# NoahVl/Explaining-In-Style-Reproducibility-Study

Hardware: AMD Instinct MI355X
Metric: StylEx G+D+enc train-step images/sec @256px (higher is better)
Workload: dtype bf16; 1 GPU; FFHQ-shaped 256x256 StylEx, batch 32/GPU, GAE=2 (noise+encoder micro-steps), GP every 4th step, ResNet-18 classifier; image_size=256, batch_per_gpu=32, start_step=0, gradient_accumulate_every=2, global_batch=32, parallelism=dp1

## Files before the change

### explaining-in-style-reproducibility-study_amd/csrc/conv_pipe.hip

```cpp
#include <hip/hip_runtime.h>
#include <stdint.h>
#include <stdlib.h>

#include "conv_prims.h"
#include "stylex_internal.h"

#ifndef PIPE_STORE_AUX
#define PIPE_STORE_AUX 0
#endif

struct StylexPipeArgs {
    int total_tiles;
    unsigned m_ntiles, m_tpi, m_tx;
    int dbg;
};

#ifdef STYLEX_PIPE_ABLATION
#define PIPE_DBG (pa.dbg)
#else
#define PIPE_DBG 0
#endif


namespace {

typedef StylexPipeArgs PipeArgs;

template <int NT>
struct PipeCfg {
    static constexpr int TH = NT == 128 ? 16 : 32;
    static constexpr int TW = 32, HWD = TW + 2, NP = (TH + 2) * HWD;
    static constexpr int H_PIECES = (NP + 31) / 32;
    static constexpr int H_STRIDE = H_PIECES * 1024;
    static constexpr int W_PIECES = 9 * NT / 32;
    static constexpr int W_STRIDE = W_PIECES * 1024;
    static constexpr int HS = 3, WS = 2;
    static constexpr int W_BASE = HS * H_STRIDE;
    static constexpr int BIAS_BASE = W_BASE + WS * W_STRIDE;
    static constexpr int DUMP_BASE = BIAS_BASE + 2048;
    static constexpr int SMEM = DUMP_BASE + 1024;
    static constexpr int HP_MAX = (H_PIECES + 7) / 8;
    static constexpr int WP_MAX = (W_PIECES + 7) / 8;
    static constexpr int RG = TH / 4;
};

__device__ __forceinline__ void lds_wait(bf16x8 (&av)[4], bf16x8 (&bv)[2]) {
    asm volatile("s_waitcnt lgkmcnt(0)" : "+v"(av[0]), "+v"(av[1]), "+v"(av[2]), "+v"(av[3]), "+v"(bv[0]), "+v"(bv[1]));
}
template <int HWD, int TAP>
__device__ __forceinline__ void tap_addr(int (&addr)[4], int a_base, unsigned& swz) {
    constexpr int kh = TAP / 3, kw = TAP % 3;
    asm volatile("" : "+v"(swz));
#pragma unroll
    for (int i = 0; i < 4; ++i) addr[i] = a_base + ((i + kh) * HWD + kw) * 32 + (int)(((swz >> ((i + kh) * 3 + kw)) & 1u) << 4);
}
template <int NT, int TAP>
__device__ __forceinline__ void load_tap(bf16x8 (&av)[4], bf16x8 (&bv)[2], const int (&addr)[4], int b_addr) {
    lds_read16<(TAP * NT) * 32>(bv[0], b_addr);
    lds_read16<(TAP * NT + 32) * 32>(bv[1], b_addr);
#pragma unroll
    for (int i = 0; i < 4; ++i) lds_read16<0>(av[i], addr[i]);
}

__device__ __forceinline__ void mfma8(f32x16 (&acc)[4][2], const bf16x8 (&av)[4], const bf16x8 (&bv)[2]) {
#pragma unroll
    for (int i = 0; i < 4; ++i)
#pragma unroll
        for (int j = 0; j < 2; ++j) mfma1(acc[i][j], bv[j], av[i]);
}

template <int NT, int EPI>
__global__ __launch_bounds__(512, 2) void conv3x3_pipe_kernel(ConvKParams p, PipeArgs pa) {
    using Cfg = PipeCfg<NT>;
    constexpr int TH = Cfg::TH, HWD = Cfg::HWD, NP = Cfg::NP, H_PIECES = Cfg::H_PIECES, H_STRIDE = Cfg::H_STRIDE;
    constexpr int W_PIECES = Cfg::W_PIECES, W_STRIDE = Cfg::W_STRIDE, W_BASE = Cfg::W_BASE;
    constexpr int HP_MAX = Cfg::HP_MAX, WP_MAX = Cfg::WP_MAX, RG = Cfg::RG;
    static_assert(WP_MAX + HP_MAX <= 9, "one DMA piece per tap");
    extern __shared__ __attribute__((aligned(16))) char smem[];
    const int tid = threadIdx.x, lane = tid & 63;
    const int wave = __builtin_amdgcn_readfirstlane(tid >> 6);
    const int H = p.Ho, W = p.Wo, C = p.Ck, N = p.N;
    const int n_tiles = N / NT;
    const int tiles_x = (W + 31) >> 5, tiles_y = (H + TH - 1) / TH;
    const int tpi = tiles_x * tiles_y;

    int xs, xn, bslot, nslots;
    xcd_tile_span(pa.total_tiles, xs, xn, bslot, nslots);
    if (bslot >= xn) return;
    for (int i = (bslot & 3) * (PIPE_DBG >> 8); i > 0; --i) __builtin_amdgcn_s_sleep(16);
    const int my_tiles = xcd_my_tiles(xn, bslot, nslots);
    const int nchunks = C >> 4;
    const int total = my_tiles * nchunks;

    auto decode = [&](int k, int& b, int& y0, int& x0, int& n0) {
        const int t = xs + bslot + k * nslots;
        int pt = fastdiv(t, pa.m_ntiles);
        n0 = (t - pt * n_tiles) * NT;
        b = fastdiv(pt, pa.m_tpi);
        pt -= b * tpi;
        const int ty = fastdiv(pt, pa.m_tx);
        y0 = ty * TH;
        x0 = (pt - ty * tiles_x) * 32;
    };

    const unsigned bytes_x = (unsigned)((long)p.B * H * W * C * 2);
    const unsigned bytes_w = (unsigned)((long)N * 9 * C * 2);
    const __amdgpu_buffer_rsrc_t rx = __builtin_amdgcn_make_buffer_rsrc(const_cast<float*>(p.a), 0, (int)bytes_x, 0x00020000);
    const __amdgpu_buffer_rsrc_t rw = __builtin_amdgcn_make_buffer_rsrc(const_cast<void*>(p.w), 0, (int)bytes_w, 0x00020000);
    constexpr unsigned OOB = 0x80000000u;

    const int lr = lane >> 1, pslot = lane & 1;
    const int half = pslot ^ ((lr >> 3) & 1);
    int h_dst[HP_MAX], w_dst[WP_MAX];
#pragma unroll
    for (int it = 0; it < HP_MAX; ++it) h_dst[it] = wave + 8 * it < H_PIECES ? (wave + 8 * it) * 1024 : -1;
    unsigned voff_h[HP_MAX];
    auto halo_voff = [&](int b, int y0, int x0) {
#pragma unroll
        for (int it = 0; it < HP_MAX; ++it) {
            const int piece = wave + 8 * it;
            const int hp = piece * 32 + lr;
            const int hh = hp / HWD, ww = hp - hh * HWD;
            const int y = y0 - 1 + hh, x = x0 - 1 + ww;
            const bool ok = piece < H_PIECES && hp < NP && y >= 0 && y < H && x >= 0 && x < W;
            voff_h[it] = ok ? ((unsigned)((b * H + y) * W + x) * (unsigned)C + (unsigned)half * 8u) * 2u : OOB;
        }
    };
    unsigned voff_w[WP_MAX];
#pragma unroll
    for (int it = 0; it < WP_MAX; ++it) {
        const int piece = wave + 8 * it;
        const int r = piece * 32 + lr;
        const int tap = r / NT, n = r - tap * NT;
        const int gt = p.flip_taps ? 8 - tap : tap;
        voff_w[it] = piece < W_PIECES ? ((unsigned)(n * 9 + gt) * (unsigned)C + (unsigned)half * 8u) * 2u : OOB;
        w_dst[it] = piece < W_PIECES ? piece * 1024 : -1;
    }
#define issue_h1(IT, STAGE, SOFF, MORE)                                                                              \
    dma16(rx, smem, h_dst[IT] >= 0 ? (STAGE) * H_STRIDE + h_dst[IT] : Cfg::DUMP_BASE, (MORE) ? voff_h[IT] : OOB, SOFF)
#define issue_w1(IT, WBUF, SOFF, MORE)                                                                               \
    dma16(rw, smem, w_dst[IT] >= 0 ? W_BASE + (WBUF) * W_STRIDE + w_dst[IT] : Cfg::DUMP_BASE, (MORE) ? voff_w[IT] : OOB, SOFF)

    const int rg = wave % RG, nh = wave / RG;
    const int li = lane & 31, lk = lane >> 5;
    const int a_row = (4 * rg) * HWD + li;
    int a_base = a_row * 32;
    unsigned swz = 0;
#pragma unroll
    for (int r = 0; r < 6; ++r)
#pragma unroll
        for (int kw = 0; kw < 3; ++kw) {
            const int t = a_row + r * HWD + kw;
            swz |= (unsigned)(((t >> 3) ^ lk) & 1) << (r * 3 + kw);
        }
    const int b_cur0 = W_BASE + (nh * 64 + li) * 32 + ((((li >> 3) ^ lk) & 1) << 4), b_cur1 = b_cur0 + W_STRIDE;

    if (EPI == 0 && (p.flags & STYLEX_EPI_BIAS) && tid < N) reinterpret_cast<float*>(smem + Cfg::BIAS_BASE)[tid] = p.bias[tid];

    f32x16 acc[4][2];
    auto zero_acc = [&]() {
#pragma unroll
        for (int i = 0; i < 4; ++i)
#pragma unroll
            for (int j = 0; j < 2; ++j)
#pragma unroll
                for (int e = 0; e < 16; ++e) acc[i][j][e] = 0.f;
    };
    zero_acc();

    const bool act = EPI == 0 && (p.flags & (STYLEX_EPI_LRELU | STYLEX_EPI_RELU)) != 0;
    const float slope = (p.flags & STYLEX_EPI_RELU) ? 0.f : 0.2f;
    const float gslope = p.res_scale;
    const bool mask_out = EPI == 0 && p.mask != nullptr;
    auto gatem = [&](unsigned u, unsigned bits) -> unsigned {
        const float a0 = __uint_as_float(u << 16), c0 = __uint_as_float(u & 0xffff0000u);
        f32x2_t t = {(bits & 1u) ? a0 : gslope * a0, (bits & 2u) ? c0 : gslope * c0};
        bf16x2_t r = __builtin_convertvector(t, bf16x2_t);
        return *reinterpret_cast<unsigned*>(&r);
    };
    auto gate2 = [&](unsigned u, unsigned g) -> unsigned {
        const float a0 = __uint_as_float(u << 16), c0 = __uint_as_float(u & 0xffff0000u);
        const float ga = __uint_as_float(g << 16), gc = __uint_as_float(g & 0xffff0000u);
        f32x2_t t = {ga > 0.f ? a0 : gslope * a0, gc > 0.f ? c0 : gslope * c0};
        bf16x2_t r = __builtin_convertvector(t, bf16x2_t);
        return *reinterpret_cast<unsigned*>(&r);
    };
    const unsigned bytes_y = (unsigned)((long)p.B * H * W * N * 2);
    const __amdgpu_buffer_rsrc_t ry = __builtin_amdgcn_make_buffer_rsrc(p.y, 0, (int)bytes_y, 0x00020000);
    const __amdgpu_buffer_rsrc_t rgate = __builtin_amdgcn_make_buffer_rsrc(const_cast<float*>(p.residual), 0, (int)bytes_y, 0x00020000);
    const __amdgpu_buffer_rsrc_t rmask = __builtin_amdgcn_make_buffer_rsrc(
        EPI == 2 ? const_cast<unsigned char*>(p.gate_mask) : p.mask, 0, (int)(bytes_y >> 4), 0x00020000);
    const unsigned rowb = (unsigned)(W * N) * 2u;
    auto pack2 = [](float a, float c) -> unsigned {
        f32x2_t t = {a, c};
        bf16x2_t r = __builtin_convertvector(t, bf16x2_t);
        return *reinterpret_cast<unsigned*>(&r);
    };
    const unsigned lane_off = (unsigned)(((4 * rg) * W + (lane & 7)) * N + nh * 64) * 2u +
                              (unsigned)(4 * ((lane >> 4) & 1) + 2 * ((lane >> 3) & 1) + (lane >> 5)) * 16u;
    const unsigned pixb8 = (unsigned)N * 16u;
    auto epilogue = [&](int b, int y0, int x0, int n0) {
        const int lh = lk;
        const int nb = n0 + nh * 64;
        const unsigned t_off = __builtin_amdgcn_readfirstlane((unsigned)((((long)(b * H + y0) * W + x0) * N + n0) * 2));
        const unsigned g_off = x0 + li < W ? (unsigned)(((4 * rg) * W + li) * N + nh * 64 + 8 * lh) * 2u : OOB;
#pragma unroll
        for (int i = 0; i < 4; ++i) {
            const bool row_ok = y0 + 4 * rg + i < H;
            const unsigned soff = t_off + i * rowb;
            u32x4 R[4];
#pragma unroll
            for (int j = 0; j < 2; ++j) {
                u32x4 gv[2];
                unsigned gm[2];
                if (EPI != 0) {
                    const unsigned voff = row_ok ? g_off : OOB;
#pragma unroll
                    for (int q = 0; q < 2; ++q) {
                        if (EPI == 1) gv[q] = __builtin_amdgcn_raw_buffer_load_b128(rgate, voff + (j * 64 + q * 32), soff, 0);
                        if (EPI == 2) gm[q] = __builtin_amdgcn_raw_buffer_load_b8(rmask, (voff >> 4) + (j * 4 + q * 2), soff >> 4, 0);
                    }
                }
                float4 b4[4];
#pragma unroll
                for (int g = 0; g < 4; ++g)
                    b4[g] = (EPI == 0 && (p.flags & STYLEX_EPI_BIAS))
                                ? *reinterpret_cast<const float4*>(smem + Cfg::BIAS_BASE + (nb + j * 32 + 8 * g + 4 * lh) * 4)
                                : make_float4(0.f, 0.f, 0.f, 0.f);
                unsigned P[4][2];
#pragma unroll
                for (int g = 0; g < 4; ++g) {
                    float v0 = acc[i][j][4 * g + 0] + b4[g].x, v1 = acc[i][j][4 * g + 1] + b4[g].y;
                    float v2 = acc[i][j][4 * g + 2] + b4[g].z, v3 = acc[i][j][4 * g + 3] + b4[g].w;
                    if (act) {
                        v0 = v0 > 0.f ? v0 : slope * v0;
                        v1 = v1 > 0.f ? v1 : slope * v1;
                        v2 = v2 > 0.f ? v2 : slope * v2;
                        v3 = v3 > 0.f ? v3 : slope * v3;
                    }
                    P[g][0] = pack2(v0, v1);
                    P[g][1] = pack2(v2, v3);
                }
#pragma unroll
                for (int g = 0; g < 4; g += 2)
#pragma unroll
                    for (int h = 0; h < 2; ++h) {
                        auto r = __builtin_amdgcn_permlane32_swap(P[g][h], P[g + 1][h], false, false);
                        P[g][h] = r[0];
                        P[g + 1][h] = r[1];
                    }
#pragma unroll
                for (int q = 0; q < 2; ++q) {
                    uint4 v = make_uint4(P[2 * q][0], P[2 * q][1], P[2 * q + 1][0], P[2 * q + 1][1]);
                    if (EPI == 1) {
                        v.x = gate2(v.x, gv[q].x);
                        v.y = gate2(v.y, gv[q].y);
                        v.z = gate2(v.z, gv[q].z);
                        v.w = gate2(v.w, gv[q].w);
                    } else if (EPI == 2) {
                        const unsigned m = gm[q];
                        v.x = gatem(v.x, m);
                        v.y = gatem(v.y, m >> 2);
                        v.z = gatem(v.z, m >> 4);
                        v.w = gatem(v.w, m >> 6);
                    }
                    if (mask_out && !(PIPE_DBG & 1))
                        __builtin_amdgcn_raw_buffer_store_b8((unsigned char)stylex_sign_bits8(v), rmask,
                                                             ((row_ok ? g_off : OOB) >> 4) + (j * 4 + q * 2), soff >> 4, 0);
                    R[2 * j + q] = u32x4{v.x, v.y, v.z, v.w};
                }
            }
#pragma unroll
            for (int j = 0; j < 2; ++j)
#pragma unroll
                for (int d = 0; d < 4; ++d) {
                    const unsigned a0 = R[2 * j][d], a1 = R[2 * j + 1][d];
                    R[2 * j][d] = (unsigned)__builtin_amdgcn_update_dpp((int)a0, (int)a1, 0x128, 0xF, 0xC, false);
                    R[2 * j + 1][d] = (unsigned)__builtin_amdgcn_update_dpp((int)a1, (int)a0, 0x128, 0xF, 0x3, false);
                }
#pragma unroll
            for (int q = 0; q < 2; ++q)
#pragma unroll
                for (int d = 0; d < 4; ++d) {
                    auto r = __builtin_amdgcn_permlane16_swap(R[q][d], R[2 + q][d], false, false);
                    R[q][d] = r[0];
                    R[2 + q][d] = r[1];
                }
            if (!(PIPE_DBG & 1)) {
#pragma unroll
                for (int k = 0; k < 4; ++k) {
                    const unsigned voff = (row_ok && x0 + 8 * k + (lane & 7) < W) ? lane_off : OOB;
                    __builtin_amdgcn_raw_buffer_store_b128(R[k], ry, voff, soff + k * pixb8, PIPE_STORE_AUX);
                    asm volatile("s_nop 1" : "+v"(R[k]) : : "memory");
                }
            }
        }
    };

    int hb, hy0, hx0, hn0;
    int h_k = 0, h_ch = 0, h_stage = 0;
    int w_k = 0, w_ch = 0, w_buf = 0, w_n0;
    int cb, cy0, cx0, cn0;
    decode(0, cb, cy0, cx0, cn0);
    hb = cb, hy0 = cy0, hx0 = cx0, hn0 = cn0;
    w_n0 = cn0;
    halo_voff(hb, hy0, hx0);
    auto adv_h = [&]() {
        h_stage = h_stage == 2 ? 0 : h_stage + 1;
        if (++h_ch == nchunks) {
            h_ch = 0;
            if (++h_k < my_tiles) {
                decode(h_k, hb, hy0, hx0, hn0);
                if (PIPE_DBG & 2) hb = 0, hy0 = 0, hx0 = 0;
                halo_voff(hb, hy0, hx0);
            }
        }
    };
    auto adv_w = [&]() {
        w_buf ^= 1;
        if (++w_ch == nchunks) {
            w_ch = 0;
            if (++w_k < my_tiles) {
                int b_, y_, x_;
                decode(w_k, b_, y_, x_, w_n0);
                if (PIPE_DBG & 4) w_n0 = 0;
            }
        }
    };
#pragma unroll
    for (int it = 0; it < HP_MAX; ++it) issue_h1(it, 0, 0u, true);
    adv_h();
#pragma unroll
    for (int it = 0; it < WP_MAX; ++it) issue_w1(it, 0, (unsigned)(w_n0 * 9 * C) * 2u, true);
    adv_w();
#pragma unroll
    for (int it = 0; it < HP_MAX; ++it) issue_h1(it, 1, (unsigned)h_ch * 32u, total > 1);
    if (total > 1) adv_h();

    int c_ch = 0, c_k = 0, c_stage = 0;
    bf16x8 avA[4], bvA[2], avB[4], bvB[2];
    int addr[4];
    tap_addr<HWD, 0>(addr, a_base, swz);
    wait_vmcnt<HP_MAX>();
    __builtin_amdgcn_s_barrier();
    asm volatile("" ::: "memory");
    load_tap<NT, 0>(avA, bvA, addr, b_cur0);
    tap_addr<HWD, 1>(addr, a_base, swz);
    auto next_stage = [&]() {
        a_base += c_stage == 2 ? -2 * H_STRIDE : H_STRIDE;
        c_stage = c_stage == 2 ? 0 : c_stage + 1;
    };
    constexpr int PPT = 2;
#define PIPE_DMA(TAP, MORE_W, MORE_H)                                                              \
    _Pragma("unroll") for (int q_ = (TAP) * PPT; q_ < (TAP) * PPT + PPT; ++q_) {                   \
        if (q_ < WP_MAX) issue_w1(q_, w_buf, w_soff, MORE_W);                                      \
        else if (q_ - WP_MAX < HP_MAX) issue_h1(q_ - WP_MAX, h_stage, h_soff, MORE_H);             \
    }
#define PIPE_TAP(TAP, AVC, BVC, AVN, BVN, BCUR, MORE_W, MORE_H) \
    lds_wait(AVC, BVC);                                        \
    load_tap<NT, TAP + 1>(AVN, BVN, addr, BCUR);               \
    __builtin_amdgcn_sched_barrier(0);                         \
    mfma8(acc, AVC, BVC);                                      \
    if (TAP == 7) next_stage();                                \
    tap_addr<HWD, (TAP + 2) % 9>(addr, a_base, swz);           \
    PIPE_DMA(TAP, MORE_W, MORE_H)                              \
    __builtin_amdgcn_sched_barrier(0);
#define PIPE_LAST(AVC, BVC, AVN, BVN, BNEXT)                   \
    lds_wait(AVC, BVC);                                        \
    if (PIPE_DBG & 8) wait_vmcnt<HP_MAX + 16>();                 \
    else wait_vmcnt<HP_MAX>();                                 \
    __builtin_amdgcn_s_barrier();                              \
    asm volatile("" ::: "memory");                             \
    load_tap<NT, 0>(AVN, BVN, addr, BNEXT);                    \
    __builtin_amdgcn_sched_barrier(0);                         \
    mfma8(acc, AVC, BVC);                                      \
    tap_addr<HWD, 1>(addr, a_base, swz);                       \
    __builtin_amdgcn_sched_barrier(0);
#define PIPE_CHUNK(A1, B1, A2, B2, BCUR, BNEXT, MORE_W, MORE_H)                                    \
    {                                                                                              \
        const bool mw_ = MORE_W, mh_ = MORE_H;                                                     \
        const unsigned w_soff = (unsigned)(w_n0 * 9 * C + w_ch * 16) * 2u, h_soff = (unsigned)h_ch * 32u; \
        PIPE_TAP(0, A1, B1, A2, B2, BCUR, mw_, mh_)                                                \
        PIPE_TAP(1, A2, B2, A1, B1, BCUR, mw_, mh_)                                                \
        PIPE_TAP(2, A1, B1, A2, B2, BCUR, mw_, mh_)                                                \
        PIPE_TAP(3, A2, B2, A1, B1, BCUR, mw_, mh_)                                                \
        PIPE_TAP(4, A1, B1, A2, B2, BCUR, mw_, mh_)                                                \
        PIPE_TAP(5, A2, B2, A1, B1, BCUR, mw_, mh_)                                                \
        PIPE_TAP(6, A1, B1, A2, B2, BCUR, mw_, mh_)                                                \
        PIPE_TAP(7, A2, B2, A1, B1, BCUR, mw_, mh_)                                                \
        PIPE_LAST(A1, B1, A2, B2, BNEXT)                                                           \
        if (mw_) adv_w();                                                                          \
        if (mh_) adv_h();                                                                          \
    }
    for (int g = 0; g < total; g += 2) {
        PIPE_CHUNK(avA, bvA, avB, bvB, b_cur0, b_cur1, g + 1 < total, g + 2 < total)
        PIPE_CHUNK(avB, bvB, avA, bvA, b_cur1, b_cur0, g + 2 < total, g + 3 < total)
        c_ch += 2;
        if (c_ch == nchunks) {
            c_ch = 0;
            asm volatile("s_nop 15\n\ts_nop 15"
                         : "+v"(acc[0][0]), "+v"(acc[0][1]), "+v"(acc[1][0]), "+v"(acc[1][1]), "+v"(acc[2][0]), "+v"(acc[2][1]),
                           "+v"(acc[3][0]), "+v"(acc[3][1]));
            epilogue(cb, cy0, cx0, cn0);
            if (++c_k < my_tiles) {
                decode(c_k, cb, cy0, cx0, cn0);
                zero_acc();
            }
        }
    }
#undef PIPE_CHUNK
#undef PIPE_LAST
#undef PIPE_TAP
#undef PIPE_DMA
#undef issue_h1
#undef issue_w1
    asm volatile("s_waitcnt lgkmcnt(0)" ::: "memory");
    wait_vmcnt<0>();
}

template <int NT, int EPI>
int launch_pipe(const ConvKParams& p, hipStream_t s) {
    using Cfg = PipeCfg<NT>;
    const hipError_t e = stylex_dynamic_lds_once<conv3x3_pipe_kernel<NT, EPI>>(Cfg::SMEM);
    if (e != hipSuccess) return (int)e;
    const int tiles_x = (p.Wo + 31) / 32, tiles_y = (p.Ho + Cfg::TH - 1) / Cfg::TH, n_tiles = p.N / NT;
    PipeArgs pa;
    pa.total_tiles = p.B * tiles_x * tiles_y * n_tiles;
    pa.m_ntiles = magic_of(n_tiles);
    pa.m_tpi = magic_of(tiles_x * tiles_y);
    pa.m_tx = magic_of(tiles_x);
#ifdef STYLEX_PIPE_ABLATION
    pa.dbg = getenv("STYLEX_PIPE_DBG") ? atoi(getenv("STYLEX_PIPE_DBG")) : 0;
#else
    pa.dbg = 0;
#endif
    stylex_note_kernel("conv3x3_pipe_kernel<%d, %d>", NT, EPI);
    hipLaunchKernelGGL((conv3x3_pipe_kernel<NT, EPI>), dim3((unsigned)stylex_cu_count()), dim3(512), Cfg::SMEM, s, p, pa);
    return (int)hipGetLastError();
}

template <int NT>
int launch_pipe_epi(const ConvKParams& p, hipStream_t s) {
    if (p.flags & STYLEX_EPI_GATE) return launch_pipe<NT, 1>(p, s);
    if (p.flags & STYLEX_EPI_GATE_MASK) return launch_pipe<NT, 2>(p, s);
    return launch_pipe<NT, 0>(p, s);
}

}

int stylex_launch_pipe(const ConvKParams& p, hipStream_t s) {
    const char* env = getenv("STYLEX_CONV_PIPE");
    if (env && env[0] == '0') return STYLEX_NOT_APPLICABLE;
    if (!p.act_bf16 || p.a_scale || p.s2d_c) return STYLEX_NOT_APPLICABLE;
    if (p.flags & ~(STYLEX_EPI_BIAS | STYLEX_EPI_LRELU | STYLEX_EPI_RELU | STYLEX_EPI_GATE | STYLEX_EPI_GATE_MASK | STYLEX_EPI_MASK_OUT))
        return STYLEX_NOT_APPLICABLE;
    if ((p.flags & STYLEX_EPI_GATE) && (!p.residual || (reinterpret_cast<uintptr_t>(p.residual) & 15))) return STYLEX_NOT_APPLICABLE;
    if (p.Ck < 64 || p.Ck % 32 != 0 || p.N % 64 != 0 || p.N > 512 || p.Wo < 32 || p.Ho < 16) return STYLEX_NOT_APPLICABLE;
    if ((reinterpret_cast<uintptr_t>(p.a) & 15) || (reinterpret_cast<uintptr_t>(p.w) & 15) || (reinterpret_cast<uintptr_t>(p.y) & 15))
        return STYLEX_NOT_APPLICABLE;
    if ((long)p.B * p.Ho * p.Wo * p.Ck * 2 >= (1l << 31) || (long)p.N * 9 * p.Ck * 2 >= (1l << 31) ||
        (long)p.B * p.Ho * p.Wo * p.N * 2 >= (1l << 31))
        return STYLEX_NOT_APPLICABLE;
    const bool n128 = p.N % 128 == 0 && !(env && env[0] == '6');
    if (!n128) {
        if (p.Ho < 32 && !(env && env[0] == '6')) return STYLEX_NOT_APPLICABLE;
        if (!(env && env[0] == '6') && ((p.flags & STYLEX_EPI_GATE) || (p.flip_taps && !p.flags && p.Ck == 64)))
            return STYLEX_NOT_APPLICABLE;
    }
    if (p.dry) return 0;
    if (n128) return launch_pipe_epi<128>(p, s);
    return launch_pipe_epi<64>(p, s);
}
```

Before: 1005 images/sec.

## Add modulated-conv path to pipelined 3x3 conv kernel with fused demod and noise epilogue

Adds a MOD variant of the pipelined 3x3 conv kernel for StyleGAN modulated convolutions. Previously these were rejected whenever a_scale was set. The new variant scales the activation halo in LDS by per-sample input scales, using a fourth halo stage to leave time for the in-place rescale. Its epilogue applies the per-output demodulation scale plus a noise injection term, reading noise tiles and scales through spare DMA slots. This routes modulated convs onto the MFMA pipeline and removes separate modulation and epilogue work, at the cost of more LDS, extra LDS round-trips per chunk, and idle waves when NT=64.

```diff
diff --git a/explaining-in-style-reproducibility-study_amd/csrc/conv_pipe.hip b/explaining-in-style-reproducibility-study_amd/csrc/conv_pipe.hip
--- a/explaining-in-style-reproducibility-study_amd/csrc/conv_pipe.hip
+++ b/explaining-in-style-reproducibility-study_amd/csrc/conv_pipe.hip
@@ -26,18 +26,21 @@
 
 typedef StylexPipeArgs PipeArgs;
 
-template <int NT>
+template <int NT, bool MOD = false>
 struct PipeCfg {
-    static constexpr int TH = NT == 128 ? 16 : 32;
+    static constexpr int TH = (NT == 128 || MOD) ? 16 : 32;
     static constexpr int TW = 32, HWD = TW + 2, NP = (TH + 2) * HWD;
     static constexpr int H_PIECES = (NP + 31) / 32;
     static constexpr int H_STRIDE = H_PIECES * 1024;
     static constexpr int W_PIECES = 9 * NT / 32;
     static constexpr int W_STRIDE = W_PIECES * 1024;
-    static constexpr int HS = 3, WS = 2;
+    static constexpr int HS = MOD ? 4 : 3, WS = 2;
     static constexpr int W_BASE = HS * H_STRIDE;
     static constexpr int BIAS_BASE = W_BASE + WS * W_STRIDE;
-    static constexpr int DUMP_BASE = BIAS_BASE + 2048;
+    static constexpr int NB_BASE = BIAS_BASE + 2048;
+    static constexpr int DTAB_BASE = NB_BASE + 2048;
+    static constexpr int NZ_BASE = DTAB_BASE + 1024;
+    static constexpr int DUMP_BASE = MOD ? NZ_BASE + 2048 : BIAS_BASE + 2048;
     static constexpr int SMEM = DUMP_BASE + 1024;
     static constexpr int HP_MAX = (H_PIECES + 7) / 8;
     static constexpr int WP_MAX = (W_PIECES + 7) / 8;
@@ -69,13 +72,30 @@
         for (int j = 0; j < 2; ++j) mfma1(acc[i][j], bv[j], av[i]);
 }
 
-template <int NT, int EPI>
+template <int OFF = 0>
+__device__ __forceinline__ void lds_read16u(u32x4& dst, int addr) {
+    asm volatile("ds_read_b128 %0, %1 offset:%2" : "=v"(dst) : "v"(addr), "n"(OFF));
+}
+__device__ __forceinline__ void lds_read4f(float& dst, int addr) { asm volatile("ds_read_b32 %0, %1" : "=v"(dst) : "v"(addr)); }
+__device__ __forceinline__ void lds_write16u(int addr, const u32x4& v) {
+    asm volatile("ds_write_b128 %0, %1" : : "v"(addr), "v"(v) : "memory");
+}
+__device__ __forceinline__ void mod_row8(u32x4& v, const float (&s)[8]) {
+#pragma unroll
+    for (int d = 0; d < 4; ++d) v[d] = act_pack2(act_lo(v[d]) * s[2 * d], act_hi(v[d]) * s[2 * d + 1]);
+}
+
+template <int NT, int EPIT>
 __global__ __launch_bounds__(512, 2) void conv3x3_pipe_kernel(ConvKParams p, PipeArgs pa) {
-    using Cfg = PipeCfg<NT>;
+    constexpr bool MOD = EPIT == 3;
+    constexpr int EPI = MOD ? 0 : EPIT;
+    using Cfg = PipeCfg<NT, MOD>;
     constexpr int TH = Cfg::TH, HWD = Cfg::HWD, NP = Cfg::NP, H_PIECES = Cfg::H_PIECES, H_STRIDE = Cfg::H_STRIDE;
     constexpr int W_PIECES = Cfg::W_PIECES, W_STRIDE = Cfg::W_STRIDE, W_BASE = Cfg::W_BASE;
-    constexpr int HP_MAX = Cfg::HP_MAX, WP_MAX = Cfg::WP_MAX, RG = Cfg::RG;
+    constexpr int HP_MAX = Cfg::HP_MAX, WP_MAX = Cfg::WP_MAX, RG = Cfg::RG, HS = Cfg::HS;
+    constexpr int HA = HS - 1;
     static_assert(WP_MAX + HP_MAX <= 9, "one DMA piece per tap");
+    static_assert(Cfg::SMEM <= 163840, "LDS of one CU");
     extern __shared__ __attribute__((aligned(16))) char smem[];
     const int tid = threadIdx.x, lane = tid & 63;
     const int wave = __builtin_amdgcn_readfirstlane(tid >> 6);
@@ -89,7 +109,8 @@
     if (bslot >= xn) return;
     for (int i = (bslot & 3) * (PIPE_DBG >> 8); i > 0; --i) __builtin_amdgcn_s_sleep(16);
     const int my_tiles = xcd_my_tiles(xn, bslot, nslots);
-    const int nchunks = C >> 4;
+#define nreal (C >> 4)
+    const int nchunks = MOD ? ((C + 31) >> 5) * 2 : C >> 4;
     const int total = my_tiles * nchunks;
 
     auto decode = [&](int k, int& b, int& y0, int& x0, int& n0) {
@@ -119,7 +140,8 @@
 #pragma unroll
         for (int it = 0; it < HP_MAX; ++it) {
             const int piece = wave + 8 * it;
-            const int hp = piece * 32 + lr;
+            int hp = piece * 32 + lr;
+            if (MOD) asm volatile("" : "+v"(hp));
             const int hh = hp / HWD, ww = hp - hh * HWD;
             const int y = y0 - 1 + hh, x = x0 - 1 + ww;
             const bool ok = piece < H_PIECES && hp < NP && y >= 0 && y < H && x >= 0 && x < W;
@@ -141,7 +163,33 @@
 #define issue_w1(IT, WBUF, SOFF, MORE)                                                                               \
     dma16(rw, smem, w_dst[IT] >= 0 ? W_BASE + (WBUF) * W_STRIDE + w_dst[IT] : Cfg::DUMP_BASE, (MORE) ? voff_w[IT] : OOB, SOFF)
 
+    static_assert(!MOD || 5 + 8 * (WP_MAX - 1) >= W_PIECES, "waves 5-7 have no weight piece in the last slot");
+    const bool has_d = MOD && (p.flags & STYLEX_EPI_OSCALE), has_nz = MOD && (p.flags & STYLEX_EPI_NOISE);
+    const bool nz_nat = MOD && (p.flags & STYLEX_EPI_NOISE_NAT) != 0;
+    const int NS = MOD ? p.noise_stride : 0;
+#define raux                                                                                                         \
+    __builtin_amdgcn_make_buffer_rsrc(wave == 7 ? const_cast<float*>(p.out_scale) : const_cast<float*>(p.noise), 0, \
+                                      wave == 7 ? p.B * N * 4 : p.B * NS * NS * 4, 0x00020000)
+    const int aux_dst = !MOD ? 0 : wave == 7 ? Cfg::DTAB_BASE : Cfg::NZ_BASE + (wave == 6 ? 1024 : 0);
+    bool aux_on = false;
+    unsigned aux_voff, aux_soff;
+#define aux_setup(b, y0, x0, n0)                                                                              \
+    if (wave == 7) {                                                                                          \
+        aux_voff = lane < NT / 4 ? (unsigned)lane * 16u : OOB;                                                \
+        aux_soff = (unsigned)((b) * N + (n0)) * 4u;                                                           \
+    } else {                                                                                                  \
+        const int q__ = wave - 5;                                                                             \
+        const int yy_ = nz_nat ? (y0) + q__ * 8 + (lane >> 3) : (y0) + 4 * (lane & 3);                        \
+        const int xx_ = nz_nat ? (x0) + 4 * (lane & 7) : (x0) + q__ * 16 + (lane >> 2);                       \
+        aux_voff = (yy_ < NS && xx_ < NS) ? (unsigned)(nz_nat ? yy_ * NS + xx_ : xx_ * NS + yy_) * 4u : OOB;  \
+        aux_soff = (unsigned)((b) * NS * NS) * 4u;                                                            \
+    }
+    const int m_half = MOD ? wave & 1 : 0;
+    const int m_off = !MOD ? 0 : (wave >> 1) * 2048 + lane * 32 + (((m_half ^ (lane >> 3)) & 1) << 4);
+
     const int rg = wave % RG, nh = wave / RG;
+    constexpr bool HALF_IDLE = MOD && NT == 64;
+#define PIPE_MM (!HALF_IDLE || nh == 0)
     const int li = lane & 31, lk = lane >> 5;
     const int a_row = (4 * rg) * HWD + li;
     int a_base = a_row * 32;
@@ -155,7 +203,15 @@
         }
     const int b_cur0 = W_BASE + (nh * 64 + li) * 32 + ((((li >> 3) ^ lk) & 1) << 4), b_cur1 = b_cur0 + W_STRIDE;
 
-    if (EPI == 0 && (p.flags & STYLEX_EPI_BIAS) && tid < N) reinterpret_cast<float*>(smem + Cfg::BIAS_BASE)[tid] = p.bias[tid];
+    if (!MOD && EPI == 0 && (p.flags & STYLEX_EPI_BIAS) && tid < N) reinterpret_cast<float*>(smem + Cfg::BIAS_BASE)[tid] = p.bias[tid];
+    if (MOD) {
+        if (tid < N) {
+            reinterpret_cast<float*>(smem + Cfg::BIAS_BASE)[tid] = has_nz ? p.noise_w[tid] : 0.f;
+            reinterpret_cast<float*>(smem + Cfg::NB_BASE)[tid] = has_nz ? p.noise_b[tid] : 0.f;
+        }
+        if (!has_nz) reinterpret_cast<float*>(smem + Cfg::NZ_BASE)[tid] = 0.f;
+        if (!has_d && tid < NT) reinterpret_cast<float*>(smem + Cfg::DTAB_BASE)[tid] = 1.f;
+    }
 
     f32x16 acc[4][2];
     auto zero_acc = [&]() {
@@ -204,8 +260,11 @@
         const int nb = n0 + nh * 64;
         const unsigned t_off = __builtin_amdgcn_readfirstlane((unsigned)((((long)(b * H + y0) * W + x0) * N + n0) * 2));
         const unsigned g_off = x0 + li < W ? (unsigned)(((4 * rg) * W + li) * N + nh * 64 + 8 * lh) * 2u : OOB;
+        const int nz_addr = !MOD ? 0 : Cfg::NZ_BASE + (nz_nat ? (4 * rg) * 32 + li : li * 16 + 4 * rg) * 4;
 #pragma unroll
         for (int i = 0; i < 4; ++i) {
+            float nzv = 0.f;
+            if (MOD) lds_read4f(nzv, nz_addr + (nz_nat ? i * 128 : i * 4));
             const bool row_ok = y0 + 4 * rg + i < H;
             const unsigned soff = t_off + i * rowb;
             u32x4 R[4];
@@ -222,16 +281,40 @@
                     }
                 }
                 float4 b4[4];
-#pragma unroll
-                for (int g = 0; g < 4; ++g)
-                    b4[g] = (EPI == 0 && (p.flags & STYLEX_EPI_BIAS))
-                                ? *reinterpret_cast<const float4*>(smem + Cfg::BIAS_BASE + (nb + j * 32 + 8 * g + 4 * lh) * 4)
-                                : make_float4(0.f, 0.f, 0.f, 0.f);
+                u32x4 dq[4], wq[4], cq[4];
+                const int ta_d = !MOD ? 0 : Cfg::DTAB_BASE + (nh * 64 + j * 32 + 4 * lh) * 4, ta_w = !MOD ? 0 : ta_d + (Cfg::BIAS_BASE - Cfg::DTAB_BASE) + n0 * 4;
+#define MOD_TABLES(G)                                                                                            \
+    {                                                                                                            \
+        lds_read16u<(G) * 32>(dq[G], ta_d);                                                                      \
+        lds_read16u<(G) * 32>(wq[G], ta_w);                                                                      \
+        lds_read16u<(G) * 32 + (Cfg::NB_BASE - Cfg::BIAS_BASE)>(cq[G], ta_w);                                    \
+        asm volatile("s_waitcnt lgkmcnt(0)" : "+v"(dq[G]), "+v"(wq[G]), "+v"(cq[G]), "+v"(nzv));                 \
+    }
+                if (!MOD) {
+#pragma unroll
+                    for (int g = 0; g < 4; ++g)
+                        b4[g] = (EPI == 0 && (p.flags & STYLEX_EPI_BIAS))
+                                    ? *reinterpret_cast<const float4*>(smem + Cfg::BIAS_BASE + (nb + j * 32 + 8 * g + 4 * lh) * 4)
+                                    : make_float4(0.f, 0.f, 0.f, 0.f);
+                }
                 unsigned P[4][2];
 #pragma unroll
                 for (int g = 0; g < 4; ++g) {
-                    float v0 = acc[i][j][4 * g + 0] + b4[g].x, v1 = acc[i][j][4 * g + 1] + b4[g].y;
-                    float v2 = acc[i][j][4 * g + 2] + b4[g].z, v3 = acc[i][j][4 * g + 3] + b4[g].w;
+                    float v0, v1, v2, v3;
+                    if (MOD) {
+                        if (g == 0) MOD_TABLES(0)
+                        if (g == 1) MOD_TABLES(1)
+                        if (g == 2) MOD_TABLES(2)
+                        if (g == 3) MOD_TABLES(3)
+                        const float z = nzv;
+                        v0 = acc[i][j][4 * g + 0] * __uint_as_float(dq[g][0]) + (z * __uint_as_float(wq[g][0]) + __uint_as_float(cq[g][0]));
+                        v1 = acc[i][j][4 * g + 1] * __uint_as_float(dq[g][1]) + (z * __uint_as_float(wq[g][1]) + __uint_as_float(cq[g][1]));
+                        v2 = acc[i][j][4 * g + 2] * __uint_as_float(dq[g][2]) + (z * __uint_as_float(wq[g][2]) + __uint_as_float(cq[g][2]));
+                        v3 = acc[i][j][4 * g + 3] * __uint_as_float(dq[g][3]) + (z * __uint_as_float(wq[g][3]) + __uint_as_float(cq[g][3]));
+                    } else {
+                        v0 = acc[i][j][4 * g + 0] + b4[g].x, v1 = acc[i][j][4 * g + 1] + b4[g].y;
+                        v2 = acc[i][j][4 * g + 2] + b4[g].z, v3 = acc[i][j][4 * g + 3] + b4[g].w;
+                    }
                     if (act) {
                         v0 = v0 > 0.f ? v0 : slope * v0;
                         v1 = v1 > 0.f ? v1 : slope * v1;
@@ -306,7 +389,7 @@
     w_n0 = cn0;
     halo_voff(hb, hy0, hx0);
     auto adv_h = [&]() {
-        h_stage = h_stage == 2 ? 0 : h_stage + 1;
+        h_stage = h_stage == HS - 1 ? 0 : h_stage + 1;
         if (++h_ch == nchunks) {
             h_ch = 0;
             if (++h_k < my_tiles) {
@@ -327,15 +410,66 @@
             }
         }
     };
+    int m_k = 0, m_ch = 0, m_b = MOD ? cb : 0, m_stage = 0;
+#define adv_m()                              \
+    {                                        \
+        m_stage = (m_stage + 1) & 3;         \
+        if (++m_ch == nchunks) {             \
+            m_ch = 0;                        \
+            if (++m_k < my_tiles) {          \
+                int y_, x_, n_;              \
+                decode(m_k, m_b, y_, x_, n_); \
+            }                                \
+        }                                    \
+    }
+    typedef unsigned u32x8 __attribute__((ext_vector_type(8)));
+    u32x8 msc;
+    u32x4 mv;
+#define mod_scales()                                                                                           \
+    {                                                                                                          \
+        const float* sp_ = p.a_scale + ((long)m_b * C + (m_ch < nreal ? m_ch : nreal - 1) * 16 + m_half * 8);  \
+        asm volatile("s_load_dwordx8 %0, %1, 0x0\n\ts_waitcnt lgkmcnt(0)" : "=&s"(msc) : "s"(sp_) : "memory"); \
+    }
+#define mod_issue(IT) \
+    if ((IT) < 2 || wave < 4) lds_read16u(mv, m_stage * H_STRIDE + m_off + (IT) * 8192);
+#define mod_finish(IT)                                                     \
+    if ((IT) < 2 || wave < 4) {                                            \
+        asm volatile("s_waitcnt lgkmcnt(0)" : "+v"(mv));                   \
+        float ms_[8];                                                      \
+        _Pragma("unroll") for (int e_ = 0; e_ < 8; ++e_) ms_[e_] = __uint_as_float(msc[e_]); \
+        mod_row8(mv, ms_);                                                 \
+        lds_write16u(m_stage * H_STRIDE + m_off + (IT) * 8192, mv);        \
+    }
+    static_assert(!MOD || H_STRIDE == 2 * 8192 + 4 * 1024, "640 rows: ten 64-row blocks, 4 per step, waves 0-3 a third step");
+
 #pragma unroll
     for (int it = 0; it < HP_MAX; ++it) issue_h1(it, 0, 0u, true);
     adv_h();
 #pragma unroll
     for (int it = 0; it < WP_MAX; ++it) issue_w1(it, 0, (unsigned)(w_n0 * 9 * C) * 2u, true);
     adv_w();
-#pragma unroll
-    for (int it = 0; it < HP_MAX; ++it) issue_h1(it, 1, (unsigned)h_ch * 32u, total > 1);
+    if (MOD) {
+        const bool real1 = total > 1 && h_ch < nreal;
+#pragma unroll
+        for (int it = 0; it < HP_MAX; ++it) issue_h1(it, 1, (unsigned)h_ch * 32u, real1);
+    } else {
+#pragma unroll
+        for (int it = 0; it < HP_MAX; ++it) issue_h1(it, 1, (unsigned)h_ch * 32u, total > 1);
+    }
     if (total > 1) adv_h();
+    if (MOD) {
+        const bool real2 = total > 2 && h_ch < nreal;
+#pragma unroll
+        for (int it = 0; it < HP_MAX; ++it) issue_h1(it, 2, (unsigned)h_ch * 32u, real2);
+        if (total > 2) adv_h();
+        wait_vmcnt<2 * HP_MAX>();
+        __builtin_amdgcn_s_barrier();
+        asm volatile("" ::: "memory");
+        mod_scales()
+        mod_issue(0) mod_finish(0) mod_issue(1) mod_finish(1) mod_issue(2) mod_finish(2)
+        adv_m()
+        asm volatile("s_waitcnt lgkmcnt(0)" ::: "memory");
+    }
 
     int c_ch = 0, c_k = 0, c_stage = 0;
     bf16x8 avA[4], bvA[2], avB[4], bvB[2];
@@ -344,64 +478,86 @@
     wait_vmcnt<HP_MAX>();
     __builtin_amdgcn_s_barrier();
     asm volatile("" ::: "memory");
-    load_tap<NT, 0>(avA, bvA, addr, b_cur0);
+    if (PIPE_MM) load_tap<NT, 0>(avA, bvA, addr, b_cur0);
     tap_addr<HWD, 1>(addr, a_base, swz);
     auto next_stage = [&]() {
-        a_base += c_stage == 2 ? -2 * H_STRIDE : H_STRIDE;
-        c_stage = c_stage == 2 ? 0 : c_stage + 1;
+        a_base += c_stage == HS - 1 ? -(HS - 1) * H_STRIDE : H_STRIDE;
+        c_stage = c_stage == HS - 1 ? 0 : c_stage + 1;
     };
     constexpr int PPT = 2;
 #define PIPE_DMA(TAP, MORE_W, MORE_H)                                                              \
     _Pragma("unroll") for (int q_ = (TAP) * PPT; q_ < (TAP) * PPT + PPT; ++q_) {                   \
-        if (q_ < WP_MAX) issue_w1(q_, w_buf, w_soff, MORE_W);                                      \
+        if (MOD && q_ == WP_MAX - 1 && aux_on) {                                                   \
+            aux_setup(cb, cy0, cx0, cn0);                                                          \
+            dma16(raux, smem, aux_dst, aux_voff, aux_soff);                                        \
+        }                                                                                          \
+        else if (q_ < WP_MAX) issue_w1(q_, w_buf, w_soff, MORE_W);                                 \
         else if (q_ - WP_MAX < HP_MAX) issue_h1(q_ - WP_MAX, h_stage, h_soff, MORE_H);             \
     }
 #define PIPE_TAP(TAP, AVC, BVC, AVN, BVN, BCUR, MORE_W, MORE_H) \
-    lds_wait(AVC, BVC);                                        \
-    load_tap<NT, TAP + 1>(AVN, BVN, addr, BCUR);               \
+    if (PIPE_MM) {                                                  \
+        lds_wait(AVC, BVC);                                    \
+        load_tap<NT, TAP + 1>(AVN, BVN, addr, BCUR);           \
+    }                                                          \
+    if (MOD && TAP >= 4 && TAP <= 6) { mod_issue(TAP - 4) }    \
     __builtin_amdgcn_sched_barrier(0);                         \
-    mfma8(acc, AVC, BVC);                                      \
+    if (PIPE_MM) mfma8(acc, AVC, BVC);                              \
+    if (MOD && TAP == 3) mod_scales()                          \
+    if (MOD && TAP >= 4 && TAP <= 6) { mod_finish(TAP - 4) }   \
     if (TAP == 7) next_stage();                                \
     tap_addr<HWD, (TAP + 2) % 9>(addr, a_base, swz);           \
     PIPE_DMA(TAP, MORE_W, MORE_H)                              \
     __builtin_amdgcn_sched_barrier(0);
 #define PIPE_LAST(AVC, BVC, AVN, BVN, BNEXT)                   \
-    lds_wait(AVC, BVC);                                        \
+    if (PIPE_MM) lds_wait(AVC, BVC);                                \
+    if (MOD) asm volatile("s_waitcnt lgkmcnt(0)" ::: "memory"); \
     if (PIPE_DBG & 8) wait_vmcnt<HP_MAX + 16>();                 \
     else wait_vmcnt<HP_MAX>();                                 \
     __builtin_amdgcn_s_barrier();                              \
     asm volatile("" ::: "memory");                             \
-    load_tap<NT, 0>(AVN, BVN, addr, BNEXT);                    \
+    if (PIPE_MM) load_tap<NT, 0>(AVN, BVN, addr, BNEXT);            \
     __builtin_amdgcn_sched_barrier(0);                         \
-    mfma8(acc, AVC, BVC);                                      \
+    if (PIPE_MM) mfma8(acc, AVC, BVC);                              \
     tap_addr<HWD, 1>(addr, a_base, swz);                       \
     __builtin_amdgcn_sched_barrier(0);
+#define PIPE_TAPS(A1, B1, A2, B2, BCUR, BNEXT, RW, RH)                                             \
+        PIPE_TAP(0, A1, B1, A2, B2, BCUR, RW, RH)                                                  \
+        PIPE_TAP(1, A2, B2, A1, B1, BCUR, RW, RH)                                                  \
+        PIPE_TAP(2, A1, B1, A2, B2, BCUR, RW, RH)                                                  \
+        PIPE_TAP(3, A2, B2, A1, B1, BCUR, RW, RH)                                                  \
+        PIPE_TAP(4, A1, B1, A2, B2, BCUR, RW, RH)                                                  \
+        PIPE_TAP(5, A2, B2, A1, B1, BCUR, RW, RH)                                                  \
+        PIPE_TAP(6, A1, B1, A2, B2, BCUR, RW, RH)                                                  \
+        PIPE_TAP(7, A2, B2, A1, B1, BCUR, RW, RH)                                                  \
+        PIPE_LAST(A1, B1, A2, B2, BNEXT)
 #define PIPE_CHUNK(A1, B1, A2, B2, BCUR, BNEXT, MORE_W, MORE_H)                                    \
     {                                                                                              \
         const bool mw_ = MORE_W, mh_ = MORE_H;                                                     \
         const unsigned w_soff = (unsigned)(w_n0 * 9 * C + w_ch * 16) * 2u, h_soff = (unsigned)h_ch * 32u; \
-        PIPE_TAP(0, A1, B1, A2, B2, BCUR, mw_, mh_)                                                \
-        PIPE_TAP(1, A2, B2, A1, B1, BCUR, mw_, mh_)                                                \
-        PIPE_TAP(2, A1, B1, A2, B2, BCUR, mw_, mh_)                                                \
-        PIPE_TAP(3, A2, B2, A1, B1, BCUR, mw_, mh_)                                                \
-        PIPE_TAP(4, A1, B1, A2, B2, BCUR, mw_, mh_)                                                \
-        PIPE_TAP(5, A2, B2, A1, B1, BCUR, mw_, mh_)                                                \
-        PIPE_TAP(6, A1, B1, A2, B2, BCUR, mw_, mh_)                                                \
-        PIPE_TAP(7, A2, B2, A1, B1, BCUR, mw_, mh_)                                                \
-        PIPE_LAST(A1, B1, A2, B2, BNEXT)                                                           \
+        if (MOD) {                                                                                 \
+            const bool mwr_ = mw_ && w_ch < nreal, mhr_ = mh_ && h_ch < nreal;                     \
+            PIPE_TAPS(A1, B1, A2, B2, BCUR, BNEXT, mwr_, mhr_)                                     \
+        } else {                                                                                   \
+            PIPE_TAPS(A1, B1, A2, B2, BCUR, BNEXT, mw_, mh_)                                       \
+        }                                                                                          \
         if (mw_) adv_w();                                                                          \
         if (mh_) adv_h();                                                                          \
+        if (MOD) adv_m()                                                                           \
     }
     for (int g = 0; g < total; g += 2) {
-        PIPE_CHUNK(avA, bvA, avB, bvB, b_cur0, b_cur1, g + 1 < total, g + 2 < total)
-        PIPE_CHUNK(avB, bvB, avA, bvA, b_cur1, b_cur0, g + 2 < total, g + 3 < total)
+        PIPE_CHUNK(avA, bvA, avB, bvB, b_cur0, b_cur1, g + 1 < total, g + HA < total)
+        if (MOD && c_ch + 2 == nchunks) {
+            aux_on = wave >= 5 && (wave == 7 ? has_d : has_nz);
+        }
+        PIPE_CHUNK(avB, bvB, avA, bvA, b_cur1, b_cur0, g + 2 < total, g + (HA + 1) < total)
+        if (MOD) aux_on = false;
         c_ch += 2;
         if (c_ch == nchunks) {
             c_ch = 0;
             asm volatile("s_nop 15\n\ts_nop 15"
                          : "+v"(acc[0][0]), "+v"(acc[0][1]), "+v"(acc[1][0]), "+v"(acc[1][1]), "+v"(acc[2][0]), "+v"(acc[2][1]),
                            "+v"(acc[3][0]), "+v"(acc[3][1]));
-            epilogue(cb, cy0, cx0, cn0);
+            if (PIPE_MM) epilogue(cb, cy0, cx0, cn0);
             if (++c_k < my_tiles) {
                 decode(c_k, cb, cy0, cx0, cn0);
                 zero_acc();
@@ -409,6 +565,7 @@
         }
     }
 #undef PIPE_CHUNK
+#undef PIPE_TAPS
 #undef PIPE_LAST
 #undef PIPE_TAP
 #undef PIPE_DMA
@@ -416,13 +573,20 @@
 #undef issue_w1
     asm volatile("s_waitcnt lgkmcnt(0)" ::: "memory");
     wait_vmcnt<0>();
-}
-
-template <int NT, int EPI>
-int launch_pipe(const ConvKParams& p, hipStream_t s) {
-    using Cfg = PipeCfg<NT>;
-    const hipError_t e = stylex_dynamic_lds_once<conv3x3_pipe_kernel<NT, EPI>>(Cfg::SMEM);
-    if (e != hipSuccess) return (int)e;
+#undef PIPE_MM
+#undef nreal
+#undef raux
+#undef mod_issue
+#undef mod_scales
+#undef adv_m
+#undef aux_setup
+#undef mod_finish
+#undef MOD_TABLES
+}
+
+template <int NT, bool MOD>
+PipeArgs pipe_args(const ConvKParams& p) {
+    using Cfg = PipeCfg<NT, MOD>;
     const int tiles_x = (p.Wo + 31) / 32, tiles_y = (p.Ho + Cfg::TH - 1) / Cfg::TH, n_tiles = p.N / NT;
     PipeArgs pa;
     pa.total_tiles = p.B * tiles_x * tiles_y * n_tiles;
@@ -434,8 +598,28 @@
 #else
     pa.dbg = 0;
 #endif
+    return pa;
+}
+
+template <int NT, int EPI>
+int launch_pipe(const ConvKParams& p, hipStream_t s) {
+    using Cfg = PipeCfg<NT>;
+    const hipError_t e = stylex_dynamic_lds_once<conv3x3_pipe_kernel<NT, EPI>>(Cfg::SMEM);
+    if (e != hipSuccess) return (int)e;
+    const PipeArgs pa = pipe_args<NT, false>(p);
     stylex_note_kernel("conv3x3_pipe_kernel<%d, %d>", NT, EPI);
     hipLaunchKernelGGL((conv3x3_pipe_kernel<NT, EPI>), dim3((unsigned)stylex_cu_count()), dim3(512), Cfg::SMEM, s, p, pa);
+    return (int)hipGetLastError();
+}
+
+template <int NT>
+int launch_pipe_mod(const ConvKParams& p, hipStream_t s) {
+    using Cfg = PipeCfg<NT, true>;
+    const hipError_t e = stylex_dynamic_lds_once<conv3x3_pipe_kernel<NT, 3>>(Cfg::SMEM);
+    if (e != hipSuccess) return (int)e;
+    const PipeArgs pa = pipe_args<NT, true>(p);
+    stylex_note_kernel("conv3x3_pipe_kernel<%d, 3>", NT);
+    hipLaunchKernelGGL((conv3x3_pipe_kernel<NT, 3>), dim3((unsigned)stylex_cu_count()), dim3(512), Cfg::SMEM, s, p, pa);
     return (int)hipGetLastError();
 }
 
@@ -446,12 +630,15 @@
     return launch_pipe<NT, 0>(p, s);
 }
 
+int launch_pipe_modulated(const ConvKParams& p, hipStream_t s);
+
 }
 
 int stylex_launch_pipe(const ConvKParams& p, hipStream_t s) {
     const char* env = getenv("STYLEX_CONV_PIPE");
     if (env && env[0] == '0') return STYLEX_NOT_APPLICABLE;
-    if (!p.act_bf16 || p.a_scale || p.s2d_c) return STYLEX_NOT_APPLICABLE;
+    if (p.a_scale) return launch_pipe_modulated(p, s);
+    if (!p.act_bf16 || p.s2d_c) return STYLEX_NOT_APPLICABLE;
     if (p.flags & ~(STYLEX_EPI_BIAS | STYLEX_EPI_LRELU | STYLEX_EPI_RELU | STYLEX_EPI_GATE | STYLEX_EPI_GATE_MASK | STYLEX_EPI_MASK_OUT))
         return STYLEX_NOT_APPLICABLE;
     if ((p.flags & STYLEX_EPI_GATE) && (!p.residual || (reinterpret_cast<uintptr_t>(p.residual) & 15))) return STYLEX_NOT_APPLICABLE;
@@ -471,3 +658,31 @@
     if (n128) return launch_pipe_epi<128>(p, s);
     return launch_pipe_epi<64>(p, s);
 }
+
+namespace {
+
+int launch_pipe_modulated(const ConvKParams& p, hipStream_t s) {
+    const char* env = getenv("STYLEX_MODCONV_PIPE");
+    if (env && env[0] == '0') return STYLEX_NOT_APPLICABLE;
+    if (!p.act_bf16 || p.s2d_c || p.flip_taps || p.transposed || p.mask || p.gate_mask || p.x2) return STYLEX_NOT_APPLICABLE;
+    if (p.flags & ~(STYLEX_EPI_OSCALE | STYLEX_EPI_NOISE | STYLEX_EPI_NOISE_NAT | STYLEX_EPI_LRELU)) return STYLEX_NOT_APPLICABLE;
+    if (p.Ck < 32 || p.Ck % 16 != 0 || p.N % 64 != 0 || p.N > 512 || p.Wo < 32 || p.Ho < 32) return STYLEX_NOT_APPLICABLE;
+    const void* al16[4] = {p.a, p.w, p.y, (p.flags & STYLEX_EPI_OSCALE) ? p.out_scale : nullptr};
+    for (const void* q : al16)
+        if (reinterpret_cast<uintptr_t>(q) & 15) return STYLEX_NOT_APPLICABLE;
+    if (reinterpret_cast<uintptr_t>(p.a_scale) & 3) return STYLEX_NOT_APPLICABLE;
+    if ((p.flags & STYLEX_EPI_OSCALE) && !p.out_scale) return STYLEX_NOT_APPLICABLE;
+    if (p.flags & STYLEX_EPI_NOISE) {
+        if (!p.noise || !p.noise_w || !p.noise_b || (reinterpret_cast<uintptr_t>(p.noise) & 15) || p.noise_stride % 4 != 0 ||
+            p.noise_stride < p.Ho || p.noise_stride < p.Wo || (long)p.B * p.noise_stride * p.noise_stride * 4 >= (1l << 31))
+            return STYLEX_NOT_APPLICABLE;
+    }
+    if ((long)p.B * p.Ho * p.Wo * p.Ck * 2 >= (1l << 31) || (long)p.N * 9 * p.Ck * 2 >= (1l << 31) ||
+        (long)p.B * p.Ho * p.Wo * p.N * 2 >= (1l << 31))
+        return STYLEX_NOT_APPLICABLE;
+    if (p.dry) return 0;
+    if (p.N % 128 == 0) return launch_pipe_mod<128>(p, s);
+    return launch_pipe_mod<64>(p, s);
+}
+
+}
```

Measured after the change: 1001 images/sec. Within noise of the previous version (-0.4%).
